# Meng-333/FastDiffSR

Hardware: AMD Instinct MI355X
Metric: 256x256 SR images/sec at T=20 (higher is better)
Workload: dtype f16x3; 1 GPU; x4 64->256, batch=16/GPU, T=20, random-init FastDiffSR UNet (inner 64, mults 1-2-4-4), 256x256, conv arithmetic f16x3 (BASELINE configs[1]); batch_per_gpu=16, global_batch=16, noise=drawn in the loop by the engine (Philox4x32-10), hipgraph=False, parallelism=dp1 (independent batches, weights broadcast once)

## Files before the change

### fastdiffsr_amd/csrc/fdsr_conv_k32.hip

```cpp
#include "fdsr_conv_dev.h"

#include <type_traits>

namespace fdsr {

#ifndef XS_F16X3
#define XS_F16X3 2
#endif
#ifndef XS_BF16
#define XS_BF16 4
#endif
#ifndef K32_PIN
#define K32_PIN 1
#endif
#ifndef K32_RIDER2
#define K32_RIDER2 1
#endif
#ifndef K32_SPLIT
#define K32_SPLIT 1
#endif
#ifndef K32_SPLIT_BF16
#define K32_SPLIT_BF16 1
#endif
#ifndef K32_MIXSPLIT
// ... 617 lines not shown
          mq[mb][ph] = *reinterpret_cast<const unsigned*>(mk + (hm ? pix * Ct + cs : (size_t)0));
        }
      }
#pragma unroll
      for (int mb = 0; mb < MB; ++mb) {
        const int oy = oy0 + wm + mb * WM;
#pragma unroll
        for (int ph = 0; ph < 2; ++ph) {
          const int ox = ox0 + 16 * ph + c15;
          const bool ok = INTERIOR || (cok[ch] && oy < p.Hout && ox < p.Wout);
          const f32x4 v = acc[mb][ph][ch] * winv + add[ch];
          const f32x4 x = xq[mb][ph];
          const unsigned m = mq[mb][ph];
          f32x4 gq, gx;
#pragma unroll
          for (int r = 0; r < 4; ++r) {
            float d = v[r];
            if (hm) d = ((m >> (8 * r)) & 0xffu) ? d * ds : 0.f;
            const float xh = (x[r] - gme[r]) * grs[r];
            float gg = d;
            if (!p.gb_plain && !(K32_GNB_DIAG & 1)) {
              const float u = fmaf(x[r], gsc[r], gsh[r]);
              const float sg = __builtin_amdgcn_rcpf(1.0f + __expf(-u));
              gg = d * (sg * (1.0f + u * (1.0f - sg)));
            }
            gq[r] = gg;
            gx[r] = gg * xh;
          }
          if (ok) {
            *reinterpret_cast<f32x4*>(p.out + obase + mb * rstride + ph * pstride + 16 * ch) = gq;
            s1[ch] += gq;
            s2[ch] += gx;
          }
        }
      }
    }
  };
  if constexpr (GNB) {
    if (interior) epilogue_gnb(std::true_type{});
    else epilogue_gnb(std::false_type{});
  } else {
    if (prec_is16(PREC) && !p.out_f32) epilogue(std::true_type{});
    else epilogue(std::false_type{});
  }
  if (p.part_out) {
    float vals[16];
#pragma unroll
    for (int ch = 0; ch < 2; ++ch)
#pragma unroll
      for (int r = 0; r < 4; ++r) { vals[ch * 8 + r * 2] = s1[ch][r]; vals[ch * 8 + r * 2 + 1] = s2[ch][r]; }
#pragma unroll
    for (int half = 8; half >= 1; half >>= 1) {
      const bool up = (c15 & half) != 0;
#pragma unroll
      for (int i = 0; i < half; ++i) {
        const float keep = up ? vals[i + half] : vals[i];
        const float send = up ? vals[i] : vals[i + half];
        vals[i] = keep + __shfl_xor(send, half, 64);
      }
    }
    float* sp = reinterpret_cast<float*>(smem_k);
    {
      const int ch = c15 >> 3, r = (c15 >> 1) & 3, st = c15 & 1;
      sp[(wm * BN + wn * 32 + 16 * ch + 4 * g + r) * 2 + st] = vals[0];
    }
    __syncthreads();
    float a_keep = 0.f, b_keep = 0.f;
    if (tid < BN && co0 + tid < p.Cout) {
      float a = 0.f, b = 0.f;
#pragma unroll
      for (int w = 0; w < WM; ++w) { a += sp[(w * BN + tid) * 2 + 0]; b += sp[(w * BN + tid) * 2 + 1]; }
      a_keep = a; b_keep = b;
      float* dst = p.part_out + (((size_t)n * (tilesX * tilesY) + ty * tilesX + tx) * p.Cout + co0 + tid) * 2;
      dst[0] = a;
      dst[1] = b;
    }
    if (p.gsum_out) {
      const float a2 = a_keep + __shfl_xor(a_keep, 1, 64), b2 = b_keep + __shfl_xor(b_keep, 1, 64);
      if (tid < BN && !(tid & 1) && co0 + tid < p.Cout) gsum_add(p.gsum_out, n, p.Cout >> 1, (co0 + tid) >> 1, xcc_id(), a2, b2);
    }
  }
}

template <int TH, int WN, int PREC>
struct ConvUp2K32Cfg {
  static constexpr int TW = 32, KC = 32;
  static constexpr int NP = PREC == PREC_F16X3 ? 2 : 1;
  static constexpr int WNP = PREC == PREC_BF16 ? 1 : 2;
  static constexpr int ROWB = 64 * NP;
  static constexpr int HH = TH + 1, HWD = TW + 2, NPIX = HH * HWD;
  static constexpr int WM = 8 / WN, BN = 32 * WN, MB = TH / WM;
  static constexpr int RPP = 512 / 8, NIN = (NPIX + RPP - 1) / RPP;
  static constexpr int BUF_BYTES = NPIX * ROWB;
  static constexpr int R = 4;
  static_assert(MB == 2, "two source rows per wave");
};

template <int TH, int WN, int PREC>
__global__ void __launch_bounds__(512, 2) conv_up2_k32_kernel(const ConvParams p) {
  using Cfg = ConvUp2K32Cfg<TH, WN, PREC>;
  constexpr int TW = Cfg::TW, KC = Cfg::KC, NP = Cfg::NP, ROWB = Cfg::ROWB, HWD = Cfg::HWD, NPIX = Cfg::NPIX;
  constexpr int WM = Cfg::WM, BN = Cfg::BN, MB = Cfg::MB, RPP = Cfg::RPP, NIN = Cfg::NIN, R = Cfg::R;

  extern __shared__ __attribute__((aligned(16))) unsigned char smem_uk[];
  unsigned char* sBuf0 = smem_uk;
  unsigned char* sBuf1 = smem_uk + Cfg::BUF_BYTES;

  const int tid = threadIdx.x, lane = tid & 63, wave = tid >> 6;
  const int wn = wave % WN, wm = wave / WN;
  const int c15 = lane & 15, g = lane >> 4;

  const int nco = p.Cout_pad / BN;
  const int tilesX = (p.Win + TW - 1) / TW, tilesY = (p.Hin + TH - 1) / TH;
  const int bid = xcd_block_id(blockIdx.x, gridDim.x);
  const int cot = bid % nco;
  int pt = bid / nco;
  const int py = pt & 1;
  pt >>= 1;
  const int tx = pt % tilesX;
  pt /= tilesX;
  const int ty = pt % tilesY;
  const int n = pt / tilesY;
  const int oy0 = ty * TH, ox0 = tx * TW, co0 = cot * BN;

  const int q = tid & 7, row0 = tid >> 3;
  int in_pix[NIN];
  unsigned skeys = 0;
#pragma unroll
  for (int i = 0; i < NIN; ++i) {
    const int pix = row0 + i * RPP;
    int v = -2;
    if (pix < NPIX) {
      const int hy = pix / HWD, hx = pix % HWD;
      const int iy = oy0 - 1 + py + hy, ix = ox0 - 1 + hx;
      const bool ok = iy >= 0 && iy < p.Hin && ix >= 0 && ix < p.Win;
      v = ok ? (n * p.Hin + iy) * p.Win + ix : -1;
      skeys |= (unsigned)k32_slot<PREC>(0, hx) << (3 * i);
    }
    in_pix[i] = v;
  }
  const int sbase = row0 * ROWB + 8 * (q & 1);
  using IO = ActIO<PREC>;
  typedef typename IO::Quad Quad;
  Quad rin[NIN];
  auto prefetch = [&](int kc) {
    const size_t coff = (size_t)kc * KC + q * 4;
#pragma unroll
    for (int i = 0; i < NIN; ++i) rin[i] = IO::load4(p.x0, (size_t)(in_pix[i] < 0 ? 0 : in_pix[i]) * p.C0 + coff);
  };
  auto stage = [&](unsigned char* buf) {
#pragma unroll
    for (int i = 0; i < NIN; ++i) {
      if (NIN * RPP > NPIX && i == NIN - 1 && row0 + i * RPP >= NPIX) continue;
      f32x4 v = IO::widen(rin[i]);
      const int sd = sbase + i * (RPP * ROWB) + 16 * ((q >> 1) ^ (int)((skeys >> (3 * i)) & 7u));
      if (PREC == PREC_F16X3) {
        if (p.sat_flag) sat_check(p.sat_flag, v, 65504.f);
        const float lim = in_pix[i] >= 0 ? 65504.f : 0.f;
#pragma unroll
        for (int e = 0; e < 4; ++e) v[e] = __builtin_amdgcn_fmed3f(v[e], -lim, lim);
        uint2 hi, lo;
        {
          const h2 h0 = {(_Float16)v[0], (_Float16)v[1]}, h1 = {(_Float16)v[2], (_Float16)v[3]};
          hi.x = __builtin_bit_cast(unsigned, h0);
          hi.y = __builtin_bit_cast(unsigned, h1);
        }
        asm("v_fma_mixlo_f16 %0, %1, -1.0, %2 op_sel:[0,0,0] op_sel_hi:[1,0,0]" : "=v"(lo.x) : "v"(hi.x), "v"(v[0]));
        asm("v_fma_mixhi_f16 %0, %1, -1.0, %2 op_sel:[1,0,0] op_sel_hi:[1,0,0]" : "+v"(lo.x) : "v"(hi.x), "v"(v[1]));
        asm("v_fma_mixlo_f16 %0, %1, -1.0, %2 op_sel:[0,0,0] op_sel_hi:[1,0,0]" : "=v"(lo.y) : "v"(hi.y), "v"(v[2]));
        asm("v_fma_mixhi_f16 %0, %1, -1.0, %2 op_sel:[1,0,0] op_sel_hi:[1,0,0]" : "+v"(lo.y) : "v"(hi.y), "v"(v[3]));
        *reinterpret_cast<uint2*>(buf + sd) = hi;
        *reinterpret_cast<uint2*>(buf + (sd ^ 64)) = lo;
      } else {
        const float keep = in_pix[i] >= 0 ? 1.f : 0.f;
        v = v * keep;
        *reinterpret_cast<uint2*>(buf + sd) = stage4_16<PREC>(v);
      }
    }
  };

  const uint4* wq = reinterpret_cast<const uint4*>(p.wq);
  const int nk = p.Cin_pad / KC, nk16 = p.Cin_pad / 16;
  uint4 Wf[R][2][NP];
  const int wlane = 32 * (g & 1) + c15;
  auto load_w = [&](int kc, int slot) {
    const uint4* src = wq + ((((((size_t)cot * nk16 + 2 * kc + (g >> 1)) * WN + wn) * 2 + py) * 8 + slot) * (Cfg::WNP * 64)) + wlane;
#pragma unroll
    for (int ch = 0; ch < 2; ++ch)
#pragma unroll
      for (int pl = 0; pl < NP; ++pl) Wf[slot % R][ch][pl] = src[pl * 64 + 16 * ch];
  };

  int xoff[3][NP];
#pragma unroll
  for (int c = 0; c < 3; ++c) {
    const int hx = c15 + c;
    xoff[c][0] = (wm * HWD + hx) * ROWB + 16 * k32_slot<PREC>(g, hx);
    if (NP == 2) xoff[c][NP - 1] = xoff[c][0] ^ 64;
  }

  f32x4 acc[MB][2][2][2];
#pragma unroll
  for (int mb = 0; mb < MB; ++mb)
#pragma unroll
    for (int px = 0; px < 2; ++px)
#pragma unroll
      for (int ph = 0; ph < 2; ++ph)
#pragma unroll
        for (int ch = 0; ch < 2; ++ch) acc[mb][px][ph][ch] = f32x4{0.f, 0.f, 0.f, 0.f};

#pragma unroll
  for (int sl = 0; sl < R; ++sl) load_w(0, sl);
  prefetch(0);
  stage(sBuf0);
  if (nk > 1) prefetch(1);
  __syncthreads();

  uint4 Xf[2][2][NP];
  const unsigned char* xptr[3][NP];
  auto load_x = [&](int xs, int slot, int mb) {
    const int a = (slot >> 1) & 1, c = (slot >> 2) + (slot & 1);
#pragma unroll
    for (int ph = 0; ph < 2; ++ph)
#pragma unroll
      for (int pl = 0; pl < NP; ++pl)
        Xf[xs][ph][pl] = *reinterpret_cast<const uint4*>(xptr[c][pl] + ((mb * WM + a) * HWD + 16 * ph) * ROWB);
  };
  auto mfma_step = [&](int xs, int slot, int mb) {
    const int px = slot >> 2, ws = slot % R;
    if (PREC == PREC_F16X3) {
#pragma unroll
      for (int ph = 0; ph < 2; ++ph)
#pragma unroll
        for (int ch = 0; ch < 2; ++ch) {
#pragma unroll
          for (int term = 0; term < 3; ++term) {
            const uint4 xv = Xf[xs][ph][term == 0 ? NP - 1 : 0];
            const uint4 wv = Wf[ws][ch][term == 1 ? NP - 1 : 0];
            acc[mb][px][ph][ch] = __builtin_amdgcn_mfma_f32_16x16x32_f16(__builtin_bit_cast(h8, wv), __builtin_bit_cast(h8, xv),
                                                                        acc[mb][px][ph][ch], 0, 0, 0);
          }
          __builtin_amdgcn_sched_barrier(0);
        }
    } else {
#pragma unroll
      for (int ph = 0; ph < 2; ++ph)
#pragma unroll
        for (int ch = 0; ch < 2; ++ch)
          acc[mb][px][ph][ch] = mfma16_k32<PREC>(Wf[ws][ch][0], Xf[xs][ph][0], acc[mb][px][ph][ch]);
    }
  };

  for (int kc = 0; kc < nk; ++kc) {
    unsigned char* cur = (kc & 1) ? sBuf1 : sBuf0;
    unsigned char* nxt = (kc & 1) ? sBuf0 : sBuf1;
    const bool more = kc + 1 < nk;
#pragma unroll
    for (int c = 0; c < 3; ++c)
#pragma unroll
      for (int pl = 0; pl < NP; ++pl) xptr[c][pl] = cur + xoff[c][pl];
    load_x(0, 0, 0);
#pragma unroll
    for (int slot = 0; slot < 8; ++slot) {
#pragma unroll
      for (int mb = 0; mb < MB; ++mb) {
        const int s = slot * MB + mb;
        if (s + 1 < 8 * MB) load_x((s + 1) & 1, (s + 1) / MB, (s + 1) % MB);
        __builtin_amdgcn_sched_barrier(0);
        mfma_step(s & 1, slot, mb);
        __builtin_amdgcn_sched_barrier(0);
      }
      if (slot + R < 8) load_w(kc, slot + R);
      else if (more) load_w(kc + 1, slot + R - 8);
      if (slot == 3 && more) {
        stage(nxt);
        if (kc + 2 < nk) prefetch(kc + 2);
      }
    }
    __syncthreads();
  }

  const int cob = co0 + wn * 32 + 4 * g;
  const float winv = p.w_inv_scale_dev ? *p.w_inv_scale_dev : p.w_inv_scale;
  f32x4 add[2];
  bool cok[2];
  const float* tembp = p.temb ? p.temb + (size_t)n * p.temb_stride + p.temb_off : p.bias;
  const float tmul = p.temb ? 1.f : 0.f;
#pragma unroll
  for (int ch = 0; ch < 2; ++ch) {
    const int co = cob + 16 * ch;
    cok[ch] = co < p.Cout;
    add[ch] = epi_add4<false>(p.bias, p.bias_r, tembp, tmul, cok[ch] ? co : 0);
  }
  f32x4 s1[2], s2[2];
#pragma unroll
  for (int ch = 0; ch < 2; ++ch) s1[ch] = s2[ch] = f32x4{0.f, 0.f, 0.f, 0.f};
  constexpr bool OUT16 = prec_is16(PREC);
#pragma unroll
  for (int mb = 0; mb < MB; ++mb)
#pragma unroll
    for (int px = 0; px < 2; ++px)
#pragma unroll
      for (int ph = 0; ph < 2; ++ph)
#pragma unroll
        for (int ch = 0; ch < 2; ++ch) {
          const int sy = oy0 + wm + mb * WM, sx = ox0 + 16 * ph + c15;
          if (cok[ch] && sy < p.Hin && sx < p.Win) {
            const size_t idx = ((size_t)(n * p.Hout + 2 * sy + py) * p.Wout + 2 * sx + px) * p.Cout + cob + 16 * ch;
            const f32x4 v = acc[mb][px][ph][ch] * winv + add[ch];
            put4<PREC, OUT16>(p.out, idx, v);
            s1[ch] += v;
            s2[ch] += v * v;
          }
        }
  if (p.part_out) {
    float vals[16];
#pragma unroll
    for (int ch = 0; ch < 2; ++ch)
#pragma unroll
      for (int r = 0; r < 4; ++r) { vals[ch * 8 + r * 2] = s1[ch][r]; vals[ch * 8 + r * 2 + 1] = s2[ch][r]; }
#pragma unroll
    for (int half = 8; half >= 1; half >>= 1) {
      const bool up = (c15 & half) != 0;
#pragma unroll
      for (int i = 0; i < half; ++i) {
        const float keep = up ? vals[i + half] : vals[i];
        const float send = up ? vals[i] : vals[i + half];
        vals[i] = keep + __shfl_xor(send, half, 64);
      }
    }
    float* sp = reinterpret_cast<float*>(smem_uk);
    {
      const int ch = c15 >> 3, r = (c15 >> 1) & 3, st = c15 & 1;
      sp[(wm * BN + wn * 32 + 16 * ch + 4 * g + r) * 2 + st] = vals[0];
    }
    __syncthreads();
    float a_keep = 0.f, b_keep = 0.f;
    if (tid < BN && co0 + tid < p.Cout) {
      float a = 0.f, b = 0.f;
#pragma unroll
      for (int w = 0; w < WM; ++w) { a += sp[(w * BN + tid) * 2 + 0]; b += sp[(w * BN + tid) * 2 + 1]; }
      a_keep = a; b_keep = b;
      float* dst = p.part_out + (((size_t)n * (tilesX * tilesY * 2) + (ty * tilesX + tx) * 2 + py) * p.Cout + co0 + tid) * 2;
      dst[0] = a;
      dst[1] = b;
    }
    if (p.gsum_out) {
      const float a2 = a_keep + __shfl_xor(a_keep, 1, 64), b2 = b_keep + __shfl_xor(b_keep, 1, 64);
      if (tid < BN && !(tid & 1) && co0 + tid < p.Cout) gsum_add(p.gsum_out, n, p.Cout >> 1, (co0 + tid) >> 1, xcc_id(), a2, b2);
    }
  }
}

bool conv_up2_k32_ok(int prec, const ConvParams& p) {
  if (!(g_tun.k32 & FDSR_K32_UP2) || !(g_tun.k32 & (prec_is16(prec) ? FDSR_K32_BF16 : FDSR_K32_F16X3))) return false;
  return p.C1 == 0 && p.C0 % 32 == 0 && p.C0 == p.Cin_pad && p.Cout % 4 == 0 && !p.gn_scale && !p.res;
}

template <int TH, int WN, int PREC>
static hipError_t launch_up2_k32_t(const ConvParams& q, int nwg, hipStream_t s) {
  using Cfg = ConvUp2K32Cfg<TH, WN, PREC>;
  hipLaunchKernelGGL((conv_up2_k32_kernel<TH, WN, PREC>), dim3(nwg), dim3(512), (size_t)2 * Cfg::BUF_BYTES, s, q);
  return hipGetLastError();
}

#define FDSR_UP2_K32_SHAPES(X) X(8, 2) X(4, 4) X(2, 8)

hipError_t launch_conv_up2_k32(int TH, int WN, int prec, const ConvParams& q, int nwg, hipStream_t s) {
#define X(TH_, WN_)                                                                                    \
  if (TH == TH_ && WN == WN_)                                                                          \
    return prec == PREC_F16X3 ? launch_up2_k32_t<TH_, WN_, PREC_F16X3>(q, nwg, s) : prec == PREC_F16 ? launch_up2_k32_t<TH_, WN_, PREC_F16>(q, nwg, s) : launch_up2_k32_t<TH_, WN_, PREC_BF16>(q, nwg, s);
  FDSR_UP2_K32_SHAPES(X)
#undef X
  return hipErrorInvalidValue;
}

#define FDSR_K32_SHAPES(X) X(16, 2) X(8, 4) X(4, 8) X(8, 2) X(4, 4) X(2, 8)

bool conv_k32_ok(int TH, int WN, int prec, const ConvParams& p) {
  if (!(g_tun.k32 & (prec_is16(prec) ? FDSR_K32_BF16 : FDSR_K32_F16X3))) return false;
  if (TH == 16 && p.xr0 && !(g_tun.k32 & FDSR_K32_RIDER_16ROW)) return false;
  if (TH * WN != 32 && !(TH * WN == 16 && (g_tun.k32 & FDSR_K32_SMALL_GRID_2ROW))) return false;
  if (WN != 2 && WN != 4 && WN != 8) return false;
  if (p.Cin_pad % 32 || (p.C0 + p.C1) != p.Cin_pad) return false;
  if (p.C1 != 0 && p.C0 % 32) return false;
  if (p.Cout % 4) return false;
  if (p.xr0) {
    if (p.nkr % 2 || (p.Cr0 + p.Cr1) != p.nkr * 16) return false;
    if (p.Cr1 != 0 && p.Cr0 % 32) return false;
  }
  return true;
}

template <int TH, int WN, int PREC, bool RIDER, int NW = 8, bool RF = (NW == 4), bool GNB = false, bool DROP = false, bool GNC = false>
static hipError_t launch_k32_t(const ConvParams& q, int nwg, hipStream_t s) {
  using Cfg = ConvK32Cfg<TH, WN, PREC, NW>;
  hipLaunchKernelGGL((conv_k32_kernel<TH, WN, PREC, RIDER, NW, RF, GNB, DROP, GNC>), dim3(nwg), dim3(Cfg::NT), (size_t)Cfg::LDS_BYTES + (GNC ? K32_GNC_LDS : 0), s, q);
  return hipGetLastError();
}

bool conv_k32_drop_ok(int prec, const ConvParams& q) {
  if (prec != PREC_F16X3 || !q.drop_mask || !q.gn_scale || q.gn_plain || q.C1 != 0 || q.ksplit > 1 || q.gb_x0) return false;
  return !q.xr0 || (g_tun.k32 & FDSR_K32_RIDER_FIRST_8WAVE);
}

static bool k32_gnb_ok(int prec, const ConvParams& q) {
  if (prec != PREC_F16X3 || !q.out_f32 || q.xr0 || q.res || q.ksplit > 1 || !q.gb_scale || !q.gb_shift || !q.gb_stats) return false;
  if (q.gb_G <= 0 || q.Cout % q.gb_G || q.Cout % 4) return false;
  return q.gb_x1 ? (q.gb_C0 % 4 == 0 && q.gb_C0 > 0 && q.gb_C0 < q.Cout) : q.gb_C0 == q.Cout;
}

static int k32_small_rows(int prec, bool rider) { return prec_is16(prec) && !rider ? 8 : 6; }

bool conv_k32_small_ok(ConvKind kind, int prec, const ConvParams& p) {
  if (!(g_tun.k32 & FDSR_K32_SMALL_WG_F16X3) || kind != CONV3_S1 || p.ksplit > 1 || p.Cout_pad != 64) return false;
  if (prec_is16(prec) && !(g_tun.k32 & FDSR_K32_SMALL_WG_BF16)) return false;
  if (p.xr0 && !(g_tun.k32 & (prec_is16(prec) ? FDSR_K32_SMALL_WG_RIDER_BF16 : FDSR_K32_SMALL_WG_RIDER_F16X3))) return false;
  if (!conv_k32_ok(8, 4, prec, p)) return false;
  const int th = k32_small_rows(prec, p.xr0 != nullptr);
  const long wgs = (long)p.N * ((p.Wout + 31) / 32) * ((p.Hout + th - 1) / th);
  return wgs >= g_tun.k32_sb_min_wgs;
}

hipError_t launch_conv_k32_small(int prec, const ConvParams& p, hipStream_t s, int* tiles) {
  const int th = k32_small_rows(prec, p.xr0 != nullptr);
  const int tilesX = (p.Wout + 31) / 32, tilesY = (p.Hout + th - 1) / th;
  if (tiles) *tiles = tilesX * tilesY;
  const int nwg = p.N * tilesX * tilesY;
  ConvParams q = p;
  q.out_bf16 = p.out_f32 ? 0 : prec_act16(prec);
  q.stagger = g_tun.k32_stagger;
  if (q.gb_x0) return k32_gnb_ok(prec, q) ? launch_k32_t<6, 2, PREC_F16X3, false, 4, true, true>(q, nwg, s) : hipErrorInvalidValue;
  if (q.drop_mask) {
    if (!conv_k32_drop_ok(prec, q)) return hipErrorInvalidValue;
    return q.xr0 ? launch_k32_t<6, 2, PREC_F16X3, true, 4, true, false, true>(q, nwg, s) : launch_k32_t<6, 2, PREC_F16X3, false, 4, true, false, true>(q, nwg, s);
  }
  if (prec == PREC_F16X3)
    return q.xr0 ? launch_k32_t<6, 2, PREC_F16X3, true, 4>(q, nwg, s) : launch_k32_t<6, 2, PREC_F16X3, false, 4>(q, nwg, s);
  if (prec == PREC_F16) return q.xr0 ? launch_k32_t<6, 2, PREC_F16, true, 4>(q, nwg, s) : launch_k32_t<8, 2, PREC_F16, false, 4>(q, nwg, s);
  return q.xr0 ? launch_k32_t<6, 2, PREC_BF16, true, 4>(q, nwg, s) : launch_k32_t<8, 2, PREC_BF16, false, 4>(q, nwg, s);
}

#define FDSR_K32_GNC_SHAPES(X) X(8, 2) X(4, 4) X(2, 8)
bool conv_k32_gnc_ok(int TH, int WN, int prec, const ConvParams& p) {
  if (TH * WN != 16 || !conv_k32_ok(TH, WN, prec, p)) return false;
  if (p.gb_x0 || p.drop_mask || p.gn_plain || (p.C0 & 1) || (p.C1 & 1)) return false;
  const int Cin = p.C0 + p.C1;
  return Cin <= K32_GNC_MAXC && p.gs_G > 0 && Cin % p.gs_G == 0 && ((Cin / p.gs_G) & 1) == 0;
}

hipError_t launch_conv_k32(int TH, int WN, int prec, const ConvParams& q, int nwg, hipStream_t s) {
  if (q.gs0) {
    if (!conv_k32_gnc_ok(TH, WN, prec, q)) return hipErrorInvalidValue;
    const bool rf = q.xr0 && q.ksplit <= 1 && (g_tun.k32 & FDSR_K32_RIDER_FIRST_8WAVE);
#define X(TH_, WN_)                                                                                                      \
    if (TH == TH_ && WN == WN_) {                                                                                        \
      if (rf) return prec == PREC_F16X3 ? launch_k32_t<TH_, WN_, PREC_F16X3, true, 8, true, false, false, true>(q, nwg, s)   \
                                        : prec == PREC_F16 ? launch_k32_t<TH_, WN_, PREC_F16, true, 8, true, false, false, true>(q, nwg, s) : launch_k32_t<TH_, WN_, PREC_BF16, true, 8, true, false, false, true>(q, nwg, s);    \
      if (q.xr0) return prec == PREC_F16X3 ? launch_k32_t<TH_, WN_, PREC_F16X3, true, 8, false, false, false, true>(q, nwg, s)  \
                                           : prec == PREC_F16 ? launch_k32_t<TH_, WN_, PREC_F16, true, 8, false, false, false, true>(q, nwg, s) : launch_k32_t<TH_, WN_, PREC_BF16, true, 8, false, false, false, true>(q, nwg, s);   \
      return prec == PREC_F16X3 ? launch_k32_t<TH_, WN_, PREC_F16X3, false, 8, false, false, false, true>(q, nwg, s)      \
                                : prec == PREC_F16 ? launch_k32_t<TH_, WN_, PREC_F16, false, 8, false, false, false, true>(q, nwg, s) : launch_k32_t<TH_, WN_, PREC_BF16, false, 8, false, false, false, true>(q, nwg, s);       \
    }
    FDSR_K32_GNC_SHAPES(X)
#undef X
    return hipErrorInvalidValue;
  }
#define X(TH_, WN_)                                                                                             \
  if (TH == TH_ && WN == WN_) {                                                                                 \
    if (q.gb_x0) return k32_gnb_ok(prec, q) ? launch_k32_t<TH_, WN_, PREC_F16X3, false, 8, false, true>(q, nwg, s) : hipErrorInvalidValue; \
    if (q.drop_mask) {                                                                                          \
      if (!conv_k32_drop_ok(prec, q)) return hipErrorInvalidValue;                                              \
      return q.xr0 ? launch_k32_t<TH_, WN_, PREC_F16X3, true, 8, true, false, true>(q, nwg, s)                  \
                   : launch_k32_t<TH_, WN_, PREC_F16X3, false, 8, false, false, true>(q, nwg, s);               \
    }                                                                                                           \
    if (q.xr0 && q.ksplit <= 1 && (g_tun.k32 & FDSR_K32_RIDER_FIRST_8WAVE))                                                           \
      return prec == PREC_F16X3 ? launch_k32_t<TH_, WN_, PREC_F16X3, true, 8, true>(q, nwg, s)                  \
                                : prec == PREC_F16 ? launch_k32_t<TH_, WN_, PREC_F16, true, 8, true>(q, nwg, s) : launch_k32_t<TH_, WN_, PREC_BF16, true, 8, true>(q, nwg, s);                  \
    if (q.xr0) return prec == PREC_F16X3 ? launch_k32_t<TH_, WN_, PREC_F16X3, true>(q, nwg, s)                  \
                                         : prec == PREC_F16 ? launch_k32_t<TH_, WN_, PREC_F16, true>(q, nwg, s) : launch_k32_t<TH_, WN_, PREC_BF16, true>(q, nwg, s);                  \
    return prec == PREC_F16X3 ? launch_k32_t<TH_, WN_, PREC_F16X3, false>(q, nwg, s)                            \
                              : prec == PREC_F16 ? launch_k32_t<TH_, WN_, PREC_F16, false>(q, nwg, s) : launch_k32_t<TH_, WN_, PREC_BF16, false>(q, nwg, s);                            \
  }
  FDSR_K32_SHAPES(X)
#undef X
  return hipErrorInvalidValue;
}

template <int TH, int WN, int PREC, bool RIDER, int NW = 8, bool RF = (NW == 4), bool GNB = false, bool DROP = false, bool GNC = false>
static hipError_t init_k32_t() {
  auto kfn = conv_k32_kernel<TH, WN, PREC, RIDER, NW, RF, GNB, DROP, GNC>;
  return hipFuncSetAttribute(reinterpret_cast<const void*>(kfn), hipFuncAttributeMaxDynamicSharedMemorySize, 160 * 1024);
}

template <int TH, int WN, int PREC>
static hipError_t init_up2_k32_t() {
  auto kfn = conv_up2_k32_kernel<TH, WN, PREC>;
  return hipFuncSetAttribute(reinterpret_cast<const void*>(kfn), hipFuncAttributeMaxDynamicSharedMemorySize, 160 * 1024);
}

hipError_t kernels_k32_init() {
  hipError_t e;
#define X(TH_, WN_)                                                                 \
  if ((e = init_up2_k32_t<TH_, WN_, PREC_F16X3>()) != hipSuccess) return e;         \
  if ((e = init_up2_k32_t<TH_, WN_, PREC_BF16>()) != hipSuccess) return e; \
  if ((e = init_up2_k32_t<TH_, WN_, PREC_F16>()) != hipSuccess) return e;
  FDSR_UP2_K32_SHAPES(X)
#undef X
#define X(TH_, WN_)                                                                        \
  if ((e = init_k32_t<TH_, WN_, PREC_F16X3, false>()) != hipSuccess) return e;             \
  if ((e = init_k32_t<TH_, WN_, PREC_F16X3, true>()) != hipSuccess) return e;              \
  if ((e = init_k32_t<TH_, WN_, PREC_BF16, false>()) != hipSuccess) return e;              \
  if ((e = init_k32_t<TH_, WN_, PREC_F16, false>()) != hipSuccess) return e;              \
  if ((e = init_k32_t<TH_, WN_, PREC_BF16, true>()) != hipSuccess) return e;                \
  if ((e = init_k32_t<TH_, WN_, PREC_F16, true>()) != hipSuccess) return e;                \
  if ((e = init_k32_t<TH_, WN_, PREC_F16X3, true, 8, true>()) != hipSuccess) return e;     \
  if ((e = init_k32_t<TH_, WN_, PREC_F16X3, false, 8, false, true>()) != hipSuccess) return e; \
  if ((e = init_k32_t<TH_, WN_, PREC_F16X3, false, 8, false, false, true>()) != hipSuccess) return e; \
  if ((e = init_k32_t<TH_, WN_, PREC_F16X3, true, 8, true, false, true>()) != hipSuccess) return e; \
  if ((e = init_k32_t<TH_, WN_, PREC_BF16, true, 8, true>()) != hipSuccess) return e; \
  if ((e = init_k32_t<TH_, WN_, PREC_F16, true, 8, true>()) != hipSuccess) return e;
  FDSR_K32_SHAPES(X)
#undef X
#define X(TH_, WN_)                                                                                                     \
  if ((e = init_k32_t<TH_, WN_, PREC_F16X3, false, 8, false, false, false, true>()) != hipSuccess) return e;            \
  if ((e = init_k32_t<TH_, WN_, PREC_F16X3, true, 8, false, false, false, true>()) != hipSuccess) return e;             \
  if ((e = init_k32_t<TH_, WN_, PREC_F16X3, true, 8, true, false, false, true>()) != hipSuccess) return e;              \
  if ((e = init_k32_t<TH_, WN_, PREC_BF16, false, 8, false, false, false, true>()) != hipSuccess) return e;             \
  if ((e = init_k32_t<TH_, WN_, PREC_F16, false, 8, false, false, false, true>()) != hipSuccess) return e;             \
  if ((e = init_k32_t<TH_, WN_, PREC_BF16, true, 8, false, false, false, true>()) != hipSuccess) return e;              \
  if ((e = init_k32_t<TH_, WN_, PREC_F16, true, 8, false, false, false, true>()) != hipSuccess) return e;              \
  if ((e = init_k32_t<TH_, WN_, PREC_BF16, true, 8, true, false, false, true>()) != hipSuccess) return e; \
  if ((e = init_k32_t<TH_, WN_, PREC_F16, true, 8, true, false, false, true>()) != hipSuccess) return e;
  FDSR_K32_GNC_SHAPES(X)
#undef X
  if ((e = init_k32_t<6, 2, PREC_F16X3, false, 4>()) != hipSuccess) return e;
  if ((e = init_k32_t<6, 2, PREC_F16X3, true, 4>()) != hipSuccess) return e;
  if ((e = init_k32_t<6, 2, PREC_F16X3, false, 4, true, true>()) != hipSuccess) return e;
  if ((e = init_k32_t<6, 2, PREC_F16X3, false, 4, true, false, true>()) != hipSuccess) return e;
  if ((e = init_k32_t<6, 2, PREC_F16X3, true, 4, true, false, true>()) != hipSuccess) return e;
  if ((e = init_k32_t<6, 2, PREC_BF16, true, 4>()) != hipSuccess) return e;
  if ((e = init_k32_t<6, 2, PREC_F16, true, 4>()) != hipSuccess) return e;
  return hipSuccess;
}

}
```

### fastdiffsr_amd/csrc/fdsr_kernels.h

```cpp
#pragma once
#include <hip/hip_runtime.h>
#include <stdint.h>
#include "../../include/fdsr.h"

namespace fdsr {

struct ConvParams {
  const float* x0;
  const float* x1;
  const float* w;
  const float* bias;
  const float* temb;
  const float* res;
  float* out;
  const float* gn_scale;
  const float* gn_shift;
  int gn_plain;
  float* part_out;
  int N, Hin, Win;
  int Hout, Wout;
  int C0, C1, Cout;
  int Cin_pad, Cout_pad;
  int temb_stride, temb_off;
  const void* wq;
  float w_inv_scale;
  const float* w_inv_scale_dev;
  int ksplit;
  float* kscratch;
  int out_f32;
  int out_bf16;
  const unsigned char* drop_mask;
  float drop_scale;
  const float* xr0;
  const float* xr1;
  int Cr0, Cr1, nkr;
  const void* wq_r;
  const float* bias_r;
  float w_inv_scale_r;
  const float* w_inv_scale_r_dev;
  int* sat_flag;
  int stagger;
  const float* gb_x0;
  const float* gb_x1;
  int gb_C0, gb_G, gb_plain;
  const float* gb_scale;
  const float* gb_shift;
  const float* gb_stats;
  const unsigned char* gb_mask;
  float gb_drop;
  unsigned long long* gsum_out;
  const unsigned long long* gs0;
  const unsigned long long* gs1;
  const float* gs_gamma;
  const float* gs_beta;
  float gs_eps;
  int gs_G;
};
enum { GSUM_SHARDS = 8, GSUM_BITS1 = 16, GSUM_BITS2 = 12 };

enum Precision { PREC_F32 = 0, PREC_F16X3 = 1, PREC_BF16 = 2, PREC_F16 = 3 };
constexpr bool prec_is16(int prec) { return prec == PREC_BF16 || prec == PREC_F16; }
constexpr int prec_wform(int prec) { return prec == PREC_F16 ? PREC_F16X3 : prec; }
constexpr int prec_act16(int prec) { return prec == PREC_BF16 ? 1 : (prec == PREC_F16 ? 2 : 0); }

struct Tunables {
  int rider = 2;
  int up2 = 1;
  long th_min_wgs = 256;
  int splitk = 1;
  int sk_target = 256;
  int wgrad_form = 0;
  int wgrad_colsum = 1;
  int wgrad_f32 = 0;
  int drop_stage = 1;
  int gnb_fuse = 1;
  long long wgrad_big_bytes = 1ll << 32;
  int k32 = FDSR_K32_DEFAULT;
  int k32_stagger = 0;
  long k32_sb_min_wgs = 1024;
  int strip = FDSR_STRIP_DEFAULT;
  long strip_min_wgs = 512;
  int tail = 1;
  int knockout = 0;
  int gn_consumer = 1;
  int bf16_f16x3_steps = 0;
  int sat_guard = 1;
  int drop_image_offset = 0;
  unsigned epoch = 0;
};
extern Tunables g_tun;
int set_tunable(const char* name, long long value);

enum ConvKind { CONV3_S1 = 0, CONV3_S2 = 1, CONV3_UP = 2, CONV1 = 3 };

void conv_tile_config(ConvKind kind, int C0, int C1, int Cout, int* KC, int* BN);
hipError_t launch_conv(ConvKind kind, const ConvParams& p, hipStream_t s, int* tiles_per_image);
hipError_t kernels_init();

void conv_h_config(ConvKind kind, int Cout, int* TH, int* WN);
hipError_t launch_conv_h(ConvKind kind, int prec, const ConvParams& p, hipStream_t s, int* tiles_per_image);
bool conv_h_gnb_ok(ConvKind kind, int prec, const ConvParams& p);
bool conv_h_drop_ok(ConvKind kind, int prec, const ConvParams& p);
bool conv_k32_drop_ok(int prec, const ConvParams& q);
int conv_h_ksplit(ConvKind kind, int N, int Hout, int Wout, int Cout, int Cout_pad, int Cin_pad, int C0, int C1);
hipError_t kernels_h_init();
bool conv_in8_ok(ConvKind kind, int prec, const ConvParams& p, int cin_real);
hipError_t launch_conv_in8(int prec, const ConvParams& p, const float* wmaster, int cin_real, hipStream_t s, int* tiles);
bool conv_out3_ok(ConvKind kind, int prec, const ConvParams& p);
hipError_t launch_conv_out3(int prec, const ConvParams& p, const float* wmaster, int cin_real, hipStream_t s, int* tiles);
hipError_t kernels_tail_init();
bool conv_k32_ok(int TH, int WN, int prec, const ConvParams& p);
hipError_t launch_conv_k32(int TH, int WN, int prec, const ConvParams& q, int nwg, hipStream_t s);
bool conv_k32_small_ok(ConvKind kind, int prec, const ConvParams& p);
bool conv_h_gnc_ok(ConvKind kind, int prec, const ConvParams& p);
bool conv_h_gsum_ok(ConvKind kind, int prec, const ConvParams& p, bool sub_pixel_up2);
bool conv_k32_gnc_ok(int TH, int WN, int prec, const ConvParams& p);
hipError_t launch_conv_k32_small(int prec, const ConvParams& p, hipStream_t s, int* tiles);
hipError_t kernels_k32_init();
bool conv_strip_ok(ConvKind kind, int prec, const ConvParams& p);
hipError_t launch_conv_strip(int prec, const ConvParams& p, int wn_a, hipStream_t s, int* tiles);
hipError_t kernels_strip_init();
bool conv_up2_k32_ok(int prec, const ConvParams& p);
hipError_t launch_conv_up2_k32(int TH, int WN, int prec, const ConvParams& q, int nwg, hipStream_t s);
hipError_t launch_conv_up2_h(int prec, const ConvParams& p, hipStream_t s, int* tiles_per_image);

struct GnFinalizeParams {
  const float* part0; int nt0, C0;
  const float* part1; int nt1, C1;
  const float* gamma; const float* beta;
  float* scale; float* shift;
  float* stats;
  const float* film;
  int film_stride, film_off;
  int N, G, HW;
  float eps;
};
hipError_t launch_gn_finalize(const GnFinalizeParams& p, hipStream_t s);
int conv_max_tiles(int H, int W);

struct TembParams {
  const float* freq;
  const float* w1;
  const float* b1;
  const float* w2;
  const float* b2;
  const float* wn;
  const float* bn;
  const float* nl_dev;
  float nl_scalar;
  float* temb;
  int inner, TE, N;
  int swish_block;
  int enc_dim, hid_dim, t_dim;
  int cos_first;
};
hipError_t launch_temb(const TembParams& p, hipStream_t s);

#define FDSR_CLAM_SLICES 32
size_t clam_slam_scratch_floats(int N, int HW, int C);
hipError_t launch_clam_gate(const float* x, int N, int HW, int C, const float* fc1 ,
                            const float* fc2 , int Cr, float* scratch, hipStream_t s, int act_bf16);
hipError_t launch_slam(const float* x, float* scratch, const float* w7 ,
                       int N, int H, int W, int C, float* out, float* part_out, hipStream_t s, int* tiles_per_image,
                       int act_bf16 );

hipError_t launch_dropout_mask(unsigned char* mask, size_t n, unsigned long long seed, unsigned step, unsigned slot, float p,
                               hipStream_t s, size_t first_elem = 0);

hipError_t launch_nchw_to_nhwc(const float* src, float* dst, int N, int Csrc, int H, int W,
                               int Cdst, int c_off, int zero_rest, hipStream_t s);
hipError_t launch_nhwc_to_nchw(const float* src, float* dst, int N, int C, int H, int W,
                               int Csrc_stride, hipStream_t s);

hipError_t launch_self_attention(const float* qkv, float* S, float* O, int N, int HW, int C, int heads, hipStream_t s, int act_bf16 = 0);
size_t attn_scratch_floats(int N, int HW, int heads);
hipError_t launch_attn_probs(const float* qkv, float* S, int N, int HW, int C, int heads, hipStream_t s);
hipError_t launch_pool2(const float* x, const float* gn_scale, const float* gn_shift, float* out, int N, int H, int W, int C,
                        hipStream_t s, int act_bf16 = 0);
hipError_t launch_upsample2(const float* x, float* out, int N, int H, int W, int C, hipStream_t s, int act_bf16 = 0);

hipError_t launch_tensor2img_u8(const float* src, unsigned char* dst, int N, int C, int H, int W, float lo, float hi,
                                hipStream_t s);

size_t image_metrics_workspace_bytes(int N, int H, int W);
hipError_t launch_image_metrics_u8(const unsigned char* a, const unsigned char* b, int N, int H, int W, int C, int flags, double* out,
                                   void* ws, hipStream_t s);
hipError_t launch_u8_to_tensor(const unsigned char* src, float* dst, int N, int C, int H, int W, float lo, float hi, hipStream_t s);

hipError_t launch_resize_bicubic_u8(const unsigned char* src, unsigned char* tmp, unsigned char* dst_u8, float* dst_f32, int N,
                                    int h, int w, int H, int W, const int* bounds_x, const int* kk_x, int ksize_x,
                                    const int* bounds_y, const int* kk_y, int ksize_y, hipStream_t s);

struct PosteriorParams {
  const float* eps;
  float* xin;
  const float* noise;
  const unsigned long long* rng;
  int rng_plane;
  float* traj;
  float* out;
  int N, HW, CP;
  float c_recip, c_recipm1, coef1, coef2, sigma;
  int plain_out;
  int x_off;
  int x0_pred;
// ... 39 lines not shown
```

### fastdiffsr_amd/csrc/fdsr_kernels.hip

```cpp
#include "fdsr_conv_dev.h"
#include "fdsr_philox.h"

#include <string>

namespace fdsr {

template <int KS, int STRIDE, bool UP, int KC, int BN, int WM>
struct ConvCfg {
  static constexpr int TH = 8, TW = 16;
  static constexpr int PAD = KS / 2;
  static constexpr int HH = (TH - 1) * STRIDE + KS;
  static constexpr int HWD = (TW - 1) * STRIDE + KS;
  static constexpr int NPIX = HH * HWD;
  static constexpr int S = KC + 4;
  static constexpr int Q = KC / 4;
  static constexpr int RPP = 256 / Q;
  static constexpr int NIN = (NPIX + RPP - 1) / RPP;
  static constexpr int WROWS = KS * KS * BN;
  static constexpr int NW = (WROWS + RPP - 1) / RPP;
  static constexpr int WN = 4 / WM;
  static constexpr int MB = 4 / WM;
  static constexpr int NB = BN / 32 / WN;
  static constexpr int LDS_FLOATS = NPIX * S + WROWS * S;
  static_assert(256 % Q == 0, "Q must divide 256");
// ... 319 lines not shown
      f_t = f[C + cc];
    }
  }
  double a = 0.0, b = 0.0;
  if (slice < S) {
    const float* part;
    int nt, Cs, cc;
    if (c < p.C0) { part = p.part0; nt = p.nt0; Cs = p.C0; cc = c; } else { part = p.part1; nt = p.nt1; Cs = p.C1; cc = c - p.C0; }
    const float* src = part + ((size_t)n * nt * Cs + cc) * 2;
    for (int t0 = slice; t0 < nt; t0 += 8 * S) {
      float2 v[8];
#pragma unroll
      for (int j = 0; j < 8; ++j) v[j] = *reinterpret_cast<const float2*>(src + (size_t)min(t0 + j * S, nt - 1) * Cs * 2);
#pragma unroll
      for (int j = 0; j < 8; ++j) {
        const bool in = t0 + j * S < nt;
        a += in ? (double)v[j].x : 0.0;
        b += in ? (double)v[j].y : 0.0;
      }
    }
  }
  sd[tid][0] = a;
  sd[tid][1] = b;
  __syncthreads();
  if (tid < 64) {
    double ga = 0.0, gb = 0.0;
#pragma unroll
    for (int k = 0; k < 4; ++k) { ga += sd[tid + 64 * k][0]; gb += sd[tid + 64 * k][1]; }
#pragma unroll
    for (int o = 32; o > 0; o >>= 1) { ga += __shfl_xor(ga, o, 64); gb += __shfl_xor(gb, o, 64); }
    if (tid == 0) {
      const double inv = 1.0 / ((double)cpg * (double)p.HW);
      const double mean = ga * inv;
      double var = gb * inv - mean * mean;
      var = var < 0.0 ? 0.0 : var;
      gs[0] = mean;
      gs[1] = 1.0 / sqrt(var + (double)p.eps);
      if (p.stats) {
        p.stats[((size_t)n * p.G + g) * 2] = (float)gs[0];
        p.stats[((size_t)n * p.G + g) * 2 + 1] = (float)gs[1];
      }
    }
  }
  __syncthreads();
  if (tid < cpg) {
    const int cc = g * cpg + tid;
    float sc = (float)gs[1] * gam;
    float sh = bet - (float)gs[0] * sc;
    if (p.film) {
      const float one_s = 1.0f + f_s;
      sc *= one_s;
      sh = sh * one_s + f_t;
    }
    p.scale[(size_t)n * C + cc] = sc;
    p.shift[(size_t)n * C + cc] = sh;
  }
}

hipError_t launch_gn_finalize(const GnFinalizeParams& p, hipStream_t s) {
  const int C = p.C0 + p.C1;
  if (C % p.G || C / p.G > 64) return hipErrorInvalidValue;
  hipLaunchKernelGGL(gn_finalize_kernel, dim3(p.N, p.G), dim3(256), 0, s, p);
  return hipGetLastError();
}

Tunables g_tun;

int set_tunable(const char* name, long long v) {
  const std::string n(name ? name : "");
  if (n == "rider") g_tun.rider = (int)v;
  else if (n == "up2") g_tun.up2 = (int)v;
  else if (n == "th_min_wgs") g_tun.th_min_wgs = (long)v;
  else if (n == "splitk") g_tun.splitk = (int)v;
  else if (n == "sk_target") g_tun.sk_target = (int)v;
  else if (n == "wgrad_form") g_tun.wgrad_form = (int)v;
  else if (n == "wgrad_colsum") g_tun.wgrad_colsum = (int)v;
  else if (n == "wgrad_f32") g_tun.wgrad_f32 = (int)v;
  else if (n == "gnb_fuse") g_tun.gnb_fuse = (int)v;
  else if (n == "drop_stage") g_tun.drop_stage = (int)v;
  else if (n == "wgrad_big_bytes") g_tun.wgrad_big_bytes = v;
  else if (n == "k32") g_tun.k32 = (int)v;
  else if (n == "k32_sb_min_wgs") g_tun.k32_sb_min_wgs = (long)v;
  else if (n == "k32_stagger") g_tun.k32_stagger = (int)v;
  else if (n == "strip") g_tun.strip = (int)v;
  else if (n == "strip_min_wgs") g_tun.strip_min_wgs = (long)v;
  else if (n == "gn_consumer") g_tun.gn_consumer = (int)v;
  else if (n == "bf16_f16x3_steps") g_tun.bf16_f16x3_steps = (int)v;
  else if (n == "sat_guard") g_tun.sat_guard = (int)v;
  else if (n == "tail") g_tun.tail = (int)v;
  else if (n == "knockout") g_tun.knockout = (int)v;
  else if (n == "drop_image_offset") g_tun.drop_image_offset = (int)v;
  else return -1;
  ++g_tun.epoch;
  return 0;
}

int conv_max_tiles(int H, int W) {
  const int a = ((H + 7) / 8) * ((W + 15) / 16), b = ((H + 1) / 2) * ((W + 31) / 32);
  return a > b ? a : b;
}

#define FDSR_TEMB_ROWS 512
__global__ void __launch_bounds__(256) temb_kernel(const TembParams p) {
  extern __shared__ __attribute__((aligned(16))) float st[];
  const int E = p.enc_dim ? p.enc_dim : p.inner, hid = p.hid_dim ? p.hid_dim : 4 * p.inner, Td = p.t_dim ? p.t_dim : p.inner;
  const int tid = threadIdx.x, n = blockIdx.x;
  float* enc = st;
  float* hbuf = st + E;
  float* tv = hbuf + hid;
  const float nl = p.nl_dev ? p.nl_dev[n] : p.nl_scalar;
  const int half = E / 2;
  for (int k = tid; k < half; k += 256) {
    const float e = nl * p.freq[k];
    enc[p.cos_first ? half + k : k] = sinf(e);
    enc[p.cos_first ? k : half + k] = cosf(e);
  }
  __syncthreads();
  for (int j = tid; j < hid; j += 256) {
    float a = p.b1[j];
    const float* w = p.w1 + (size_t)j * E;
    for (int k = 0; k < E; ++k) a = fmaf(w[k], enc[k], a);
    hbuf[j] = a / (1.0f + expf(-a));
  }
  __syncthreads();
  for (int j = tid; j < Td; j += 256) {
    float a = p.b2[j];
    const float* w = p.w2 + (size_t)j * hid;
    for (int k = 0; k < hid; ++k) a = fmaf(w[k], hbuf[k], a);
    tv[j] = p.swish_block ? a / (1.0f + expf(-a)) : a;
  }
  __syncthreads();
  const int o_end = min(p.TE, (int)(blockIdx.y + 1) * FDSR_TEMB_ROWS);
  for (int o = blockIdx.y * FDSR_TEMB_ROWS + tid; o < o_end; o += 256) {
    float a = p.bn[o];
    const float* w = p.wn + (size_t)o * Td;
    for (int k = 0; k < Td; ++k) a = fmaf(w[k], tv[k], a);
    p.temb[(size_t)n * p.TE + o] = a;
  }
}

hipError_t launch_temb(const TembParams& p, hipStream_t s) {
  const int E = p.enc_dim ? p.enc_dim : p.inner, hid = p.hid_dim ? p.hid_dim : 4 * p.inner, Td = p.t_dim ? p.t_dim : p.inner;
  hipLaunchKernelGGL(temb_kernel, dim3(p.N, (p.TE + FDSR_TEMB_ROWS - 1) / FDSR_TEMB_ROWS), dim3(256), (size_t)(E + hid + Td) * sizeof(float), s, p);
  return hipGetLastError();
}

__device__ __forceinline__ float wave_sum(float v) {
#pragma unroll
  for (int o = 32; o > 0; o >>= 1) v += __shfl_xor(v, o, 64);
  return v;
}
__device__ __forceinline__ float wave_max(float v) {
#pragma unroll
  for (int o = 32; o > 0; o >>= 1) v = fmaxf(v, __shfl_xor(v, o, 64));
  return v;
}

template <int BF>
__device__ __forceinline__ f32x4 ldq(const float* base, size_t idx) {
  if (BF == 2) return ActIO<PREC_F16>::widen(ActIO<PREC_F16>::load4(base, idx));
  if (BF) {
    const uint2 q = *reinterpret_cast<const uint2*>(reinterpret_cast<const unsigned short*>(base) + idx);
    f32x4 r = {__builtin_bit_cast(float, q.x << 16), __builtin_bit_cast(float, q.x & 0xffff0000u),
               __builtin_bit_cast(float, q.y << 16), __builtin_bit_cast(float, q.y & 0xffff0000u)};
    return r;
  }
// ... 772 lines not shown
```

Baseline: 72.22 images/s.

## Compute both sub-pixel row parities per workgroup in up2 conv, reusing staged input

Adds a PAIR variant of the sub-pixel up2 k32 conv in which each workgroup computes both output row parities (py=0 and py=1). The first pass stages every Cin chunk into its own LDS buffer, holding the whole input tile plus one extra halo row. The second pass reuses that LDS content with no restaging, prefetching or barriers, then emits GroupNorm partials for both parities. This halves the grid and avoids loading and staging the same input tile twice. The cost is much larger LDS use (all K chunks resident), which may lower occupancy, and the two parities now run serially inside one workgroup.

```diff
diff --git a/fastdiffsr_amd/csrc/fdsr_conv_k32.hip b/fastdiffsr_amd/csrc/fdsr_conv_k32.hip
--- a/fastdiffsr_amd/csrc/fdsr_conv_k32.hip
+++ b/fastdiffsr_amd/csrc/fdsr_conv_k32.hip
@@ -723,13 +723,13 @@
   }
 }
 
-template <int TH, int WN, int PREC>
+template <int TH, int WN, int PREC, bool PAIR = false>
 struct ConvUp2K32Cfg {
   static constexpr int TW = 32, KC = 32;
   static constexpr int NP = PREC == PREC_F16X3 ? 2 : 1;
   static constexpr int WNP = PREC == PREC_BF16 ? 1 : 2;
   static constexpr int ROWB = 64 * NP;
-  static constexpr int HH = TH + 1, HWD = TW + 2, NPIX = HH * HWD;
+  static constexpr int HH = TH + 1 + (PAIR ? 1 : 0), HWD = TW + 2, NPIX = HH * HWD;
   static constexpr int WM = 8 / WN, BN = 32 * WN, MB = TH / WM;
   static constexpr int RPP = 512 / 8, NIN = (NPIX + RPP - 1) / RPP;
   static constexpr int BUF_BYTES = NPIX * ROWB;
@@ -737,9 +737,9 @@
   static_assert(MB == 2, "two source rows per wave");
 };
 
-template <int TH, int WN, int PREC>
+template <int TH, int WN, int PREC, bool PAIR = false>
 __global__ void __launch_bounds__(512, 2) conv_up2_k32_kernel(const ConvParams p) {
-  using Cfg = ConvUp2K32Cfg<TH, WN, PREC>;
+  using Cfg = ConvUp2K32Cfg<TH, WN, PREC, PAIR>;
   constexpr int TW = Cfg::TW, KC = Cfg::KC, NP = Cfg::NP, ROWB = Cfg::ROWB, HWD = Cfg::HWD, NPIX = Cfg::NPIX;
   constexpr int WM = Cfg::WM, BN = Cfg::BN, MB = Cfg::MB, RPP = Cfg::RPP, NIN = Cfg::NIN, R = Cfg::R;
 
@@ -756,8 +756,8 @@
   const int bid = xcd_block_id(blockIdx.x, gridDim.x);
   const int cot = bid % nco;
   int pt = bid / nco;
-  const int py = pt & 1;
-  pt >>= 1;
+  const int py = PAIR ? 0 : (pt & 1);
+  if (!PAIR) pt >>= 1;
   const int tx = pt % tilesX;
   pt /= tilesX;
   const int ty = pt % tilesY;
@@ -824,8 +824,8 @@
   const int nk = p.Cin_pad / KC, nk16 = p.Cin_pad / 16;
   uint4 Wf[R][2][NP];
   const int wlane = 32 * (g & 1) + c15;
-  auto load_w = [&](int kc, int slot) {
-    const uint4* src = wq + ((((((size_t)cot * nk16 + 2 * kc + (g >> 1)) * WN + wn) * 2 + py) * 8 + slot) * (Cfg::WNP * 64)) + wlane;
+  auto load_w = [&](int pyc, int kc, int slot) {
+    const uint4* src = wq + ((((((size_t)cot * nk16 + 2 * kc + (g >> 1)) * WN + wn) * 2 + pyc) * 8 + slot) * (Cfg::WNP * 64)) + wlane;
 #pragma unroll
     for (int ch = 0; ch < 2; ++ch)
 #pragma unroll
@@ -851,7 +851,7 @@
         for (int ch = 0; ch < 2; ++ch) acc[mb][px][ph][ch] = f32x4{0.f, 0.f, 0.f, 0.f};
 
 #pragma unroll
-  for (int sl = 0; sl < R; ++sl) load_w(0, sl);
+  for (int sl = 0; sl < R; ++sl) load_w(py, 0, sl);
   prefetch(0);
   stage(sBuf0);
   if (nk > 1) prefetch(1);
@@ -892,69 +892,74 @@
     }
   };
 
-  for (int kc = 0; kc < nk; ++kc) {
-    unsigned char* cur = (kc & 1) ? sBuf1 : sBuf0;
-    unsigned char* nxt = (kc & 1) ? sBuf0 : sBuf1;
-    const bool more = kc + 1 < nk;
-#pragma unroll
-    for (int c = 0; c < 3; ++c)
-#pragma unroll
-      for (int pl = 0; pl < NP; ++pl) xptr[c][pl] = cur + xoff[c][pl];
-    load_x(0, 0, 0);
-#pragma unroll
-    for (int slot = 0; slot < 8; ++slot) {
-#pragma unroll
-      for (int mb = 0; mb < MB; ++mb) {
-        const int s = slot * MB + mb;
-        if (s + 1 < 8 * MB) load_x((s + 1) & 1, (s + 1) / MB, (s + 1) % MB);
-        __builtin_amdgcn_sched_barrier(0);
-        mfma_step(s & 1, slot, mb);
-        __builtin_amdgcn_sched_barrier(0);
-      }
-      if (slot + R < 8) load_w(kc, slot + R);
-      else if (more) load_w(kc + 1, slot + R - 8);
-      if (slot == 3 && more) {
-        stage(nxt);
-        if (kc + 2 < nk) prefetch(kc + 2);
-      }
-    }
-    __syncthreads();
-  }
-
-  const int cob = co0 + wn * 32 + 4 * g;
-  const float winv = p.w_inv_scale_dev ? *p.w_inv_scale_dev : p.w_inv_scale;
-  f32x4 add[2];
-  bool cok[2];
-  const float* tembp = p.temb ? p.temb + (size_t)n * p.temb_stride + p.temb_off : p.bias;
-  const float tmul = p.temb ? 1.f : 0.f;
-#pragma unroll
-  for (int ch = 0; ch < 2; ++ch) {
-    const int co = cob + 16 * ch;
-    cok[ch] = co < p.Cout;
-    add[ch] = epi_add4<false>(p.bias, p.bias_r, tembp, tmul, cok[ch] ? co : 0);
-  }
-  f32x4 s1[2], s2[2];
-#pragma unroll
-  for (int ch = 0; ch < 2; ++ch) s1[ch] = s2[ch] = f32x4{0.f, 0.f, 0.f, 0.f};
-  constexpr bool OUT16 = prec_is16(PREC);
-#pragma unroll
-  for (int mb = 0; mb < MB; ++mb)
-#pragma unroll
-    for (int px = 0; px < 2; ++px)
-#pragma unroll
-      for (int ph = 0; ph < 2; ++ph)
-#pragma unroll
-        for (int ch = 0; ch < 2; ++ch) {
-          const int sy = oy0 + wm + mb * WM, sx = ox0 + 16 * ph + c15;
-          if (cok[ch] && sy < p.Hin && sx < p.Win) {
-            const size_t idx = ((size_t)(n * p.Hout + 2 * sy + py) * p.Wout + 2 * sx + px) * p.Cout + cob + 16 * ch;
-            const f32x4 v = acc[mb][px][ph][ch] * winv + add[ch];
-            put4<PREC, OUT16>(p.out, idx, v);
-            s1[ch] += v;
-            s2[ch] += v * v;
+  auto k_loop = [&](const int pyc, auto staged) {
+    constexpr bool STAGED = decltype(staged)::value;
+    for (int kc = 0; kc < nk; ++kc) {
+      unsigned char* cur = PAIR ? smem_uk + kc * Cfg::BUF_BYTES : ((kc & 1) ? sBuf1 : sBuf0);
+      unsigned char* nxt = PAIR ? cur + Cfg::BUF_BYTES : ((kc & 1) ? sBuf0 : sBuf1);
+      const bool more = kc + 1 < nk;
+#pragma unroll
+      for (int c = 0; c < 3; ++c)
+#pragma unroll
+        for (int pl = 0; pl < NP; ++pl) xptr[c][pl] = cur + xoff[c][pl] + (PAIR && !STAGED ? HWD * ROWB : 0);
+      load_x(0, 0, 0);
+#pragma unroll
+      for (int slot = 0; slot < 8; ++slot) {
+#pragma unroll
+        for (int mb = 0; mb < MB; ++mb) {
+          const int s = slot * MB + mb;
+          if (s + 1 < 8 * MB) load_x((s + 1) & 1, (s + 1) / MB, (s + 1) % MB);
+          __builtin_amdgcn_sched_barrier(0);
+          mfma_step(s & 1, slot, mb);
+          __builtin_amdgcn_sched_barrier(0);
+        }
+        if (slot + R < 8) load_w(pyc, kc, slot + R);
+        else if (more) load_w(pyc, kc + 1, slot + R - 8);
+        else if (PAIR && STAGED) load_w(1, 0, slot + R - 8);
+        if (STAGED && slot == 3 && more) {
+          stage(nxt);
+          if (kc + 2 < nk) prefetch(kc + 2);
+        }
+      }
+      if (STAGED && (!PAIR || more)) __syncthreads();
+    }
+  };
+
+  auto tile_out = [&](const int pyc, f32x4 (&s1)[2], f32x4 (&s2)[2]) {
+    const int cob = co0 + wn * 32 + 4 * g;
+    const float winv = p.w_inv_scale_dev ? *p.w_inv_scale_dev : p.w_inv_scale;
+    f32x4 add[2];
+    bool cok[2];
+    const float* tembp = p.temb ? p.temb + (size_t)n * p.temb_stride + p.temb_off : p.bias;
+    const float tmul = p.temb ? 1.f : 0.f;
+#pragma unroll
+    for (int ch = 0; ch < 2; ++ch) {
+      const int co = cob + 16 * ch;
+      cok[ch] = co < p.Cout;
+      add[ch] = epi_add4<false>(p.bias, p.bias_r, tembp, tmul, cok[ch] ? co : 0);
+    }
+#pragma unroll
+    for (int ch = 0; ch < 2; ++ch) s1[ch] = s2[ch] = f32x4{0.f, 0.f, 0.f, 0.f};
+    constexpr bool OUT16 = prec_is16(PREC);
+#pragma unroll
+    for (int mb = 0; mb < MB; ++mb)
+#pragma unroll
+      for (int px = 0; px < 2; ++px)
+#pragma unroll
+        for (int ph = 0; ph < 2; ++ph)
+#pragma unroll
+          for (int ch = 0; ch < 2; ++ch) {
+            const int sy = oy0 + wm + mb * WM, sx = ox0 + 16 * ph + c15;
+            if (cok[ch] && sy < p.Hin && sx < p.Win) {
+              const size_t idx = ((size_t)(n * p.Hout + 2 * sy + pyc) * p.Wout + 2 * sx + px) * p.Cout + cob + 16 * ch;
+              const f32x4 v = acc[mb][px][ph][ch] * winv + add[ch];
+              put4<PREC, OUT16>(p.out, idx, v);
+              s1[ch] += v;
+              s2[ch] += v * v;
+            }
           }
-        }
-  if (p.part_out) {
+  };
+  auto fold = [&](const f32x4 (&s1)[2], const f32x4 (&s2)[2]) -> float {
     float vals[16];
 #pragma unroll
     for (int ch = 0; ch < 2; ++ch)
@@ -970,25 +975,60 @@
         vals[i] = keep + __shfl_xor(send, half, 64);
       }
     }
+    return vals[0];
+  };
+
+  auto tile_stat = [&](const int pyc) -> float {
+    f32x4 s1[2], s2[2];
+    tile_out(pyc, s1, s2);
+    return p.part_out ? fold(s1, s2) : 0.f;
+  };
+
+  float stat[PAIR ? 2 : 1];
+  if constexpr (PAIR) {
+    k_loop(0, std::true_type{});
+    stat[0] = tile_stat(0);
+#pragma unroll
+    for (int mb = 0; mb < MB; ++mb)
+#pragma unroll
+      for (int px = 0; px < 2; ++px)
+#pragma unroll
+        for (int ph = 0; ph < 2; ++ph)
+#pragma unroll
+          for (int ch = 0; ch < 2; ++ch) acc[mb][px][ph][ch] = f32x4{0.f, 0.f, 0.f, 0.f};
+    k_loop(1, std::false_type{});
+    stat[1] = tile_stat(1);
+  } else {
+    k_loop(py, std::true_type{});
+    stat[0] = tile_stat(py);
+  }
+  if (p.part_out) {
+    constexpr int NPY = PAIR ? 2 : 1;
+    if (PAIR) __syncthreads();
     float* sp = reinterpret_cast<float*>(smem_uk);
     {
       const int ch = c15 >> 3, r = (c15 >> 1) & 3, st = c15 & 1;
-      sp[(wm * BN + wn * 32 + 16 * ch + 4 * g + r) * 2 + st] = vals[0];
+#pragma unroll
+      for (int i = 0; i < NPY; ++i) sp[((i * WM + wm) * BN + wn * 32 + 16 * ch + 4 * g + r) * 2 + st] = stat[i];
     }
     __syncthreads();
-    float a_keep = 0.f, b_keep = 0.f;
-    if (tid < BN && co0 + tid < p.Cout) {
-      float a = 0.f, b = 0.f;
-#pragma unroll
-      for (int w = 0; w < WM; ++w) { a += sp[(w * BN + tid) * 2 + 0]; b += sp[(w * BN + tid) * 2 + 1]; }
-      a_keep = a; b_keep = b;
-      float* dst = p.part_out + (((size_t)n * (tilesX * tilesY * 2) + (ty * tilesX + tx) * 2 + py) * p.Cout + co0 + tid) * 2;
-      dst[0] = a;
-      dst[1] = b;
-    }
-    if (p.gsum_out) {
-      const float a2 = a_keep + __shfl_xor(a_keep, 1, 64), b2 = b_keep + __shfl_xor(b_keep, 1, 64);
-      if (tid < BN && !(tid & 1) && co0 + tid < p.Cout) gsum_add(p.gsum_out, n, p.Cout >> 1, (co0 + tid) >> 1, xcc_id(), a2, b2);
+#pragma unroll
+    for (int i = 0; i < NPY; ++i) {
+      const int pyc = PAIR ? i : py;
+      float a_keep = 0.f, b_keep = 0.f;
+      if (tid < BN && co0 + tid < p.Cout) {
+        float a = 0.f, b = 0.f;
+#pragma unroll
+        for (int w = 0; w < WM; ++w) { a += sp[((i * WM + w) * BN + tid) * 2 + 0]; b += sp[((i * WM + w) * BN + tid) * 2 + 1]; }
+        a_keep = a; b_keep = b;
+        float* dst = p.part_out + (((size_t)n * (tilesX * tilesY * 2) + (ty * tilesX + tx) * 2 + pyc) * p.Cout + co0 + tid) * 2;
+        dst[0] = a;
+        dst[1] = b;
+      }
+      if (p.gsum_out) {
+        const float a2 = a_keep + __shfl_xor(a_keep, 1, 64), b2 = b_keep + __shfl_xor(b_keep, 1, 64);
+        if (tid < BN && !(tid & 1) && co0 + tid < p.Cout) gsum_add(p.gsum_out, n, p.Cout >> 1, (co0 + tid) >> 1, xcc_id(), a2, b2);
+      }
     }
   }
 }
@@ -998,8 +1038,22 @@
   return p.C1 == 0 && p.C0 % 32 == 0 && p.C0 == p.Cin_pad && p.Cout % 4 == 0 && !p.gn_scale && !p.res;
 }
 
+bool conv_up2_k32_pair_ok(int prec, int Cin, int Cout, int TH, int N, int Hin, int Win) {
+  if (!g_tun.up2_pair || (TH != 8 && TH != 4 && TH != 2) || Cin <= 0 || Cin % 32) return false;
+  const int BN = 32 * (16 / TH), rowb = prec == PREC_F16X3 ? 128 : 64;
+  const long lds = (long)(Cin / 32) * (TH + 2) * 34 * rowb;
+  if (lds > 160 * 1024) return false;
+  const long wgs = (long)N * ((Win + 31) / 32) * ((Hin + TH - 1) / TH) * ((Cout + BN - 1) / BN);
+  return wgs >= g_tun.up2_pair_min_wgs;
+}
+
 template <int TH, int WN, int PREC>
 static hipError_t launch_up2_k32_t(const ConvParams& q, int nwg, hipStream_t s) {
+  if (conv_up2_k32_pair_ok(PREC, q.Cin_pad, q.Cout, TH, q.N, q.Hin, q.Win)) {
+    using Cfg = ConvUp2K32Cfg<TH, WN, PREC, true>;
+    hipLaunchKernelGGL((conv_up2_k32_kernel<TH, WN, PREC, true>), dim3(nwg / 2), dim3(512), (size_t)(q.Cin_pad / 32) * Cfg::BUF_BYTES, s, q);
+    return hipGetLastError();
+  }
   using Cfg = ConvUp2K32Cfg<TH, WN, PREC>;
   hipLaunchKernelGGL((conv_up2_k32_kernel<TH, WN, PREC>), dim3(nwg), dim3(512), (size_t)2 * Cfg::BUF_BYTES, s, q);
   return hipGetLastError();
@@ -1137,7 +1191,10 @@
 template <int TH, int WN, int PREC>
 static hipError_t init_up2_k32_t() {
   auto kfn = conv_up2_k32_kernel<TH, WN, PREC>;
-  return hipFuncSetAttribute(reinterpret_cast<const void*>(kfn), hipFuncAttributeMaxDynamicSharedMemorySize, 160 * 1024);
+  auto kfn_pair = conv_up2_k32_kernel<TH, WN, PREC, true>;
+  const hipError_t e = hipFuncSetAttribute(reinterpret_cast<const void*>(kfn), hipFuncAttributeMaxDynamicSharedMemorySize, 160 * 1024);
+  if (e != hipSuccess) return e;
+  return hipFuncSetAttribute(reinterpret_cast<const void*>(kfn_pair), hipFuncAttributeMaxDynamicSharedMemorySize, 160 * 1024);
 }
 
 hipError_t kernels_k32_init() {
diff --git a/fastdiffsr_amd/csrc/fdsr_kernels.h b/fastdiffsr_amd/csrc/fdsr_kernels.h
--- a/fastdiffsr_amd/csrc/fdsr_kernels.h
+++ b/fastdiffsr_amd/csrc/fdsr_kernels.h
@@ -78,6 +78,8 @@
   int k32 = FDSR_K32_DEFAULT;
   int k32_stagger = 0;
   long k32_sb_min_wgs = 1024;
+  int up2_pair = 1;
+  long up2_pair_min_wgs = 256;
   int strip = FDSR_STRIP_DEFAULT;
   long strip_min_wgs = 512;
   int tail = 1;
@@ -121,6 +123,7 @@
 hipError_t launch_conv_strip(int prec, const ConvParams& p, int wn_a, hipStream_t s, int* tiles);
 hipError_t kernels_strip_init();
 bool conv_up2_k32_ok(int prec, const ConvParams& p);
+bool conv_up2_k32_pair_ok(int prec, int Cin, int Cout, int TH, int N, int Hin, int Win);
 hipError_t launch_conv_up2_k32(int TH, int WN, int prec, const ConvParams& q, int nwg, hipStream_t s);
 hipError_t launch_conv_up2_h(int prec, const ConvParams& p, hipStream_t s, int* tiles_per_image);
 
diff --git a/fastdiffsr_amd/csrc/fdsr_kernels.hip b/fastdiffsr_amd/csrc/fdsr_kernels.hip
--- a/fastdiffsr_amd/csrc/fdsr_kernels.hip
+++ b/fastdiffsr_amd/csrc/fdsr_kernels.hip
@@ -425,6 +425,8 @@
   else if (n == "k32") g_tun.k32 = (int)v;
   else if (n == "k32_sb_min_wgs") g_tun.k32_sb_min_wgs = (long)v;
   else if (n == "k32_stagger") g_tun.k32_stagger = (int)v;
+  else if (n == "up2_pair") g_tun.up2_pair = (int)v;
+  else if (n == "up2_pair_min_wgs") g_tun.up2_pair_min_wgs = (long)v;
   else if (n == "strip") g_tun.strip = (int)v;
   else if (n == "strip_min_wgs") g_tun.strip_min_wgs = (long)v;
   else if (n == "gn_consumer") g_tun.gn_consumer = (int)v;
```

Measured after the change: 72.70 images/s, median of 6. No clear change (+0.7%).
